# mpieva/mapping-iterative-assembler

Measured on AMD Instinct MI355X. Metric: reads aligned/sec per iteration (16.5kb mito ref, 100bp reads), higher is better.
Workload: dtype int32; 1 GPU; configs[1]: 1000000 synthetic 100 bp reads per GPU vs mt311 (16619 bp, circular), matrix flat; step = reiterate_assembly + pop_smp + cull + consensus; pass-1 coordinates = true positions; reads_per_gpu=1000000, total_reads=1000000, consensus_len=16619, bytes_per_read=182

## Files before the change

mapping-iterative-assembler_amd/csrc/mia_hip.hip:

```cpp
#include <hip/hip_runtime.h>
#include <atomic>
#include <hip/hip_ext.h>
#include <stdio.h>
#include <stdlib.h>
#include <string.h>

#include <algorithm>
#include <cmath>
#include <chrono>
#include <string>
#include <thread>
#include <vector>

#include "../../include/mia_hip.h"
#include "mia_comm.h"
#include "mia_consensus_kernels.h"
#include "mia_kernels.h"
#include "bandx_kernels.h"
#include "mia_pass1_kernels.h"
#include "mia_myers_kernels.h"
#include "mia_trim_kernels.h"
#include "mia_peak_kernels.h"
#include "mia_iter_kernels.h"

using namespace mia;

enum Stage { STG_TRACE = 0, STG_PLAIN, STG_FILTER, STG_BAND, STG_BX_PLAN, STG_BX_VALUES, STG_BX_TRACE, STG_TALLY, STG_PASS1, STG_COUNT };
static const char* const STAGE_NAMES[STG_COUNT] = {"k_align_quad", "k_align_quad_plain", "k_diag_filter", "k_band_align", "k_bx_plan",
                                                   "k_bx_values", "k_bx_trace", "k_tally_binned", "k_pass1"};

constexpr int OPEN_WGS = 1024;
constexpr int64_t OPEN_SLAB_BYTES = (int64_t)MAX_READ * 64 * 12;
constexpr int CTRL_BINS = 0;
constexpr int CTRL_HDR = (3 * N_BINS + 2 + 1) & ~1;
constexpr int CTRL_FILTER = CTRL_HDR + PH_WORDS;
constexpr int CTRL_LKN = CTRL_FILTER + 4, CTRL_CULLF = CTRL_LKN + 1, CTRL_NEV = CTRL_CULLF + 1, CTRL_TFLAGS = CTRL_NEV + 1, CTRL_FIXN = CTRL_TFLAGS + 1;
constexpr int CTRL_GENN = CTRL_FIXN + 1;
constexpr int CTRL_BXC = (CTRL_GENN + 1 + 63) & ~63;
constexpr int CTRL_WORDS = CTRL_BXC + BXC_WORDS;
constexpr int CTRL_C0 = CTRL_BINS + 3 * N_BINS, CTRL_CN = CTRL_WORDS - CTRL_C0;

#ifdef MIA_HIP_ALT_PATHS
static inline const char* alt_env(const char* name) { return getenv(name); }
#define ALT_KERNEL(k) ((const void*)(k))
#else
static inline const char* alt_env(const char*) { return nullptr; }
#define ALT_KERNEL(k) ((const void*)nullptr)
#endif

struct mia_hip_ctx {
  int device = 0;
  int32_t* d_ctrl = nullptr;
  uint32_t stage_mask = ~0u;
  hipStream_t stream = nullptr;
  hipStream_t stream2 = nullptr; hipEvent_t ev_fork = nullptr, ev_join = nullptr;
  hipStream_t stream3 = nullptr; hipEvent_t ev_join3 = nullptr;
  int32_t* d_retry2 = nullptr; int64_t retry2_cap = 0;
  uint32_t* d_bx_slabs_late = nullptr; int64_t bx_slab_late_cap = 0; int bx_late_wgs = 0;
  uint32_t* d_bx_slabs_late2 = nullptr; bool dp_aside = false;
  const int32_t* abort_if = nullptr;
  bool spec_ok = false, spec_pending = false, spec_filtered = false, spec_bx = false, spec_plain = false;
  int64_t spec_redone = 0;
  bool pend_encode = false; int32_t pend_L = 0, pend_wl = 0, pend_total = 0;
  uint32_t* d_prep_bar = nullptr; uint32_t prep_bar_count = 0; bool no_prep_fuse = false;
  KbPair* d_kbits = nullptr;
  int use_quick = 1; int64_t quick_steps = 0;
  bool direct_open_now = false;
  int32_t* d_open_list = nullptr; int64_t open_cap = 0; unsigned char* d_slabs_open = nullptr; bool use_direct_open = true; int64_t direct_open_steps = 0;
  bool spec_force = false; int32_t* d_one = nullptr;
  bool zero_copy = true;
  bool cull_scan = false, tail_scans = false, stage_markers = false;
  bool spin_wait = true;
  uint32_t ext_events = 31u; bool planner_end_signalled = false, align_end_signalled = false;
  BxCandRec* d_bx_cand2 = nullptr; int use_fine = 1;
  BxCandRec* d_bx_cand = nullptr; int64_t cand_cap = 0, cand2_cap = 0; bool plan_split = true;
  bool no_spec = false;
  bool no_side_buckets = false;
  int buckets_queued = 0;
  hipStream_t stream4 = nullptr; hipEvent_t ev_early = nullptr;
  hipEvent_t ev_snap = nullptr, ev_v1 = nullptr; uint32_t* d_bx_snap = nullptr; int split_dp_mode = 0;
  bool cull_with_records = true;
  int64_t split_dp_steps = 0;
  bool use_early = false, early_queued = false;
  int early_wgs_per_cu = 2;
  uint8_t* d_early = nullptr; int32_t* d_trec_early = nullptr; int32_t* d_order_e = nullptr; int32_t* d_fix_list = nullptr; int64_t early_cap = 0;
  int32_t* d_bucket_e = nullptr; int bucket_e_cap = 0, bucket_e_clean_nb = -1;
  int32_t* d_tally_slabs_e = nullptr; int64_t tally_slab_e_cap = 0;
  unsigned char* d_slabs_retry[3] = {nullptr, nullptr, nullptr};
  bool bx_planner_aside = false;
  bool bx_pending_join = false;
  std::string err;
// ... 227 lines not shown
    const char* npl = alt_env("MIA_HIP_NO_PLAIN");
    if (npl && atoi(npl)) ctx->use_plain = 0;
    const char* pbb = alt_env("MIA_HIP_PLAIN_BEHIND_BAND");
    if (pbb && atoi(pbb)) ctx->plain_behind_band = 1;
    const char* nf = alt_env("MIA_HIP_NO_DIAG_FILTER");
    if (nf && atoi(nf)) { ctx->use_filter = 0; ctx->use_bx = 0; }
    const char* nbd = alt_env("MIA_HIP_NO_BAND_DP");
    if (nbd && atoi(nbd)) { ctx->use_banddp = 0; ctx->use_bx = 0; }
    const char* nbx = alt_env("MIA_HIP_NO_BANDX");
    if (nbx && atoi(nbx)) ctx->use_bx = 0;
    if (const char* nl2 = alt_env("MIA_HIP_NO_LANES")) if (atoi(nl2)) ctx->use_lanes = 0;
    if (const char* bd2 = alt_env("MIA_HIP_BX_DEBUG")) ctx->bx_dbg = (uint32_t)atoi(bd2);
    if (const char* bs2 = alt_env("MIA_HIP_BX_SERIAL")) ctx->bx_serial = atoi(bs2) != 0;
    if (const char* sb2 = alt_env("MIA_HIP_NO_SIDE_BUCKETS")) ctx->no_side_buckets = atoi(sb2) != 0;
    if (const char* ns2 = alt_env("MIA_HIP_NO_SPEC")) ctx->no_spec = atoi(ns2) != 0;
    if (const char* pf2 = alt_env("MIA_HIP_NO_PREP_FUSE")) ctx->no_prep_fuse = atoi(pf2) != 0;
    if (const char* ps2 = alt_env("MIA_HIP_NO_PLAN_SPLIT")) ctx->plan_split = atoi(ps2) == 0;
    if (const char* zc = alt_env("MIA_HIP_NO_ZERO_COPY")) ctx->zero_copy = atoi(zc) == 0;
    if (const char* ef = alt_env("MIA_HIP_NO_EXT_EVENTS")) ctx->ext_events = atoi(ef) ? 0u : 31u;
    if (const char* cs = alt_env("MIA_HIP_CULL_SCAN")) ctx->cull_scan = atoi(cs) != 0;
    if (const char* sm = alt_env("MIA_HIP_STAGE_MARKERS")) ctx->stage_markers = atoi(sm) != 0;
    if (const char* ts = alt_env("MIA_HIP_TAIL_SCANS")) ctx->tail_scans = atoi(ts) != 0;
    if (const char* dop = alt_env("MIA_HIP_NO_DIRECT_OPEN")) ctx->use_direct_open = atoi(dop) == 0;
    if (const char* qp = alt_env("MIA_HIP_NO_QUICK_PLAN")) ctx->use_quick = atoi(qp) == 0 ? 1 : 0;
    if (const char* qp = alt_env("MIA_HIP_QUICK_PLAN")) ctx->use_quick = atoi(qp);
    if (const char* sw = getenv("MIA_HIP_SPIN_WAIT")) ctx->spin_wait = atoi(sw) != 0;
    if (const char* em = alt_env("MIA_HIP_EXT_EVENTS_MASK")) ctx->ext_events = (uint32_t)atoi(em);
    if (const char* st2 = alt_env("MIA_HIP_SPEC_TEST")) ctx->spec_force = atoi(st2) != 0;
    if (const char* ml = alt_env("MIA_HIP_MYERS_NO_LANES")) ctx->myers_no_lanes = atoi(ml) != 0;
    if (const char* mo = alt_env("MIA_HIP_MYERS_NO_OND")) ctx->myers_no_ond = atoi(mo) != 0;
    if (const char* fo = alt_env("MIA_HIP_FAKE_EVENT_OVERFLOW")) ctx->fake_event_overflow = atoi(fo) != 0;
    if (const char* na = alt_env("MIA_HIP_NO_AUTO_PLAIN")) ctx->no_auto_plain = atoi(na) != 0;
    const char* egs = alt_env("MIA_HIP_EAGER_SCRIPTS");
    if (egs && atoi(egs)) ctx->lazy_scripts = 0;
    const char* nwl = alt_env("MIA_HIP_NO_WILD");
    if (nwl && atoi(nwl)) ctx->use_wild = 0;
    if (const char* ne = alt_env("MIA_HIP_EARLY_TALLY")) ctx->use_early = atoi(ne) != 0;
    if (const char* ti = alt_env("MIA_HIP_TALLY_INLINE")) ctx->tally_defer = atoi(ti) == 0;
    if (const char* ss = alt_env("MIA_HIP_STRAND_SPLIT")) ctx->tally_strand_split = atoi(ss) != 0;
    if (const char* nr = alt_env("MIA_HIP_NO_TALLY_RUNS")) ctx->tally_runs = atoi(nr) == 0;
    if (const char* sd = alt_env("MIA_HIP_SPLIT_DP")) ctx->split_dp_mode = atoi(sd) != 0 ? 1 : -1;
    if (const char* ra = alt_env("MIA_HIP_NO_TALLY_RALL")) ctx->tally_rall = atoi(ra) == 0;
    if (const char* cr = alt_env("MIA_HIP_NO_CULL_RECORDS")) ctx->cull_with_records = atoi(cr) == 0;
    if (const char* tc = alt_env("MIA_HIP_TALLY_CHUNK")) { const int c = atoi(tc); if (c == 256 || c == 512 || c == 768) ctx->tally_chunk_linear = c; }
    if (const char* ew = alt_env("MIA_HIP_EARLY_WGS")) ctx->early_wgs_per_cu = atoi(ew);
    if (const char* nf = alt_env("MIA_HIP_NO_FINE")) ctx->use_fine = atoi(nf) == 0 ? 1 : 0;
// ... 398 lines not shown
  return MIA_HIP_OK;
}

#ifdef MIA_HIP_ALT_PATHS
extern "C" int mia_hip_debug_tally_kinds(mia_hip_ctx* ctx, uint64_t* out8) {
  if (!ctx || !out8) return MIA_HIP_ERR_ARG;
  HIPCHK(hipStreamSynchronize(ctx->stream));
  HIPCHK(hipMemcpyFromSymbol(out8, HIP_SYMBOL(g_tally_kinds), 8 * sizeof(uint64_t)));
  uint64_t z[8] = {0, 0, 0, 0, 0, 0, 0, 0};
  HIPCHK(hipMemcpyToSymbol(HIP_SYMBOL(g_tally_kinds), z, sizeof z));
  HIPCHK(hipMemcpyFromSymbol(out8 + 8, HIP_SYMBOL(g_tally_clk), 8 * sizeof(uint64_t)));
  HIPCHK(hipMemcpyToSymbol(HIP_SYMBOL(g_tally_clk), z, sizeof z));
  return MIA_HIP_OK;
}
extern "C" int mia_hip_debug_plan_clk(mia_hip_ctx* ctx, uint64_t* out12) {
  if (!ctx || !out12) return MIA_HIP_ERR_ARG;
  HIPCHK(hipStreamSynchronize(ctx->stream));
  static uint64_t all[64 * 16], z[64 * 16];
  HIPCHK(hipMemcpyFromSymbol(all, HIP_SYMBOL(g_plan_clk), sizeof all));
  for (int k = 0; k < 12; k++) { out12[k] = 0; for (int st = 0; st < 64; st++) out12[k] += all[st * 16 + k]; }
  HIPCHK(hipMemcpyToSymbol(HIP_SYMBOL(g_plan_clk), z, sizeof z));
  return MIA_HIP_OK;
}
#endif
extern "C" int mia_hip_bx_counters(mia_hip_ctx* ctx, uint32_t* out32) {
  if (!ctx || !out32) return MIA_HIP_ERR_ARG;
  for (int k = 0; k < 32; k++) out32[k] = ctx->bx_last[k];
  return MIA_HIP_OK;
}

extern "C" int mia_hip_plain_stats(mia_hip_ctx* ctx, int reset, double* plain_ms, int64_t* plain_launches, int64_t* reads_in, int64_t* reads_retried) {
  if (!ctx) return MIA_HIP_ERR_ARG;
  HIPCHK(hipSetDevice(ctx->device));
  drain_events(ctx);
  if (plain_ms) *plain_ms = ctx->stg[STG_PLAIN].ms;
  if (plain_launches) *plain_launches = ctx->stg[STG_PLAIN].launches;
  if (reads_in) *reads_in = ctx->plain_total;
  if (reads_retried) *reads_retried = ctx->plain_retried;
  if (reset) { ctx->stg[STG_PLAIN].ms = 0; ctx->stg[STG_PLAIN].launches = 0; ctx->plain_total = 0; ctx->plain_retried = 0; }
  return MIA_HIP_OK;
}

template <int CPL>
static hipError_t launch_window(mia_hip_ctx* ctx, int ci, const int32_t* list, int count, const int32_t* dev_range = nullptr, hipStream_t on = nullptr,
                                bool own_slabs = false, hipEvent_t stop = nullptr) {
  const int64_t slab = (int64_t)MAX_READ * 64 * CPL;
// ... 2 lines not shown
    const int cus = ctx->cus;
    if (hipOccupancyMaxActiveBlocksPerMultiprocessor(&occ, (const void*)k_align_window<CPL>, 64, 0) != hipSuccess || occ < 1) occ = 1;
    const int per_cu = ctx->grid_wgs / cus;
    ctx->window_wgs[ci] = cus * (occ < per_cu ? occ : per_cu);
  }
  int grid = (dev_range || count >= ctx->window_wgs[ci]) ? ctx->window_wgs[ci] : count;
  unsigned char* slabs = nullptr;
  if (own_slabs) {
    grid = std::min(grid, 1024);
    if (!ctx->d_slabs_retry[ci] && hipMalloc((void**)&ctx->d_slabs_retry[ci], (size_t)slab * 1024) != hipSuccess) return hipErrorOutOfMemory;
    slabs = ctx->d_slabs_retry[ci];
  } else {
    if (!ctx->d_slabs[ci]) {
      if (hipMalloc((void**)&ctx->d_slabs[ci], (size_t)slab * ctx->grid_wgs) != hipSuccess) return hipErrorOutOfMemory;
    }
    slabs = ctx->d_slabs[ci];
  }
  RefInfo ref{ctx->d_ref, ctx->L, ctx->wrap, ctx->explicit_win};
  if (stage_begin(ctx, STG_TRACE, on)) return hipErrorOutOfMemory;
  launch_k(k_align_window<CPL>, dim3(grid), dim3(64), 0, on ? on : ctx->stream, stop, ctx->rs, ref, ctx->d_pssm, ctx->packs.p[ci], list,
           count, slabs, slab, ctx->d_wide_list, ctx->d_bins + 3 * N_BINS, ctx->dbg, dev_range);
  stage_end(ctx, STG_TRACE, on);
  return hipGetLastError();
}

static int bx_join_and_retry(mia_hip_ctx* ctx) {
  if (!ctx->bx_pending_join) return MIA_HIP_OK;
  ctx->bx_pending_join = false;
  const int32_t* range = ctx->d_plan_hdr + PH_RETRY2;
  const int cols = ctx->max_len + 2 * REALIGN_BUFFER + 2;
  const bool aside = ctx->bx_planner_aside;
  if (!aside || ctx->dp_aside) HIPCHK(hipStreamWaitEvent(ctx->stream, ctx->ev_join, 0));
  HIPCHK(hipStreamWaitEvent(ctx->stream, ctx->ev_join3, 0));
  hipEvent_t stop = (aside && (ctx->ext_events & 8u)) ? ctx->ev_fork : nullptr;
  ctx->align_end_signalled = stop != nullptr;
  hipError_t e;
  if (ctx->direct_open_now) {
    RefInfo ref{ctx->d_ref, ctx->L, ctx->wrap, ctx->explicit_win};
    if (stage_begin(ctx, STG_TRACE)) return MIA_HIP_ERR_NOMEM;
    launch_k(k_align_open, dim3(OPEN_WGS), dim3(64), 0, ctx->stream, stop, ctx->rs, ref, (const int32_t*)ctx->d_pssm, ctx->packs, (const int32_t*)ctx->d_open_list,
             (const uint32_t*)(ctx->d_bx_ctr + (size_t)BXC_OPEN * BXC_STRIDE), ctx->d_slabs_open, (int64_t)OPEN_SLAB_BYTES, ctx->d_wide_list, ctx->d_bins + 3 * N_BINS, ctx->dbg,
             (const int32_t*)ctx->d_retry2, (const uint32_t*)(range + 1));
    stage_end(ctx, STG_TRACE);
    e = hipGetLastError();
    if (e != hipSuccess) { ctx->err = std::string("k_align_open launch: ") + hipGetErrorString(e); return MIA_HIP_ERR_DEVICE; }
    return MIA_HIP_OK;
  }
  e = cols <= 64 * 4 ? launch_window<4>(ctx, 0, ctx->d_retry2, 0, range, nullptr, aside, stop)
    : cols <= 64 * 8 ? launch_window<8>(ctx, 1, ctx->d_retry2, 0, range, nullptr, aside, stop)
                     : launch_window<12>(ctx, 2, ctx->d_retry2, 0, range, nullptr, aside, stop);
  if (e != hipSuccess) { ctx->err = std::string("k_align_window (band retry list) launch: ") + hipGetErrorString(e); return MIA_HIP_ERR_DEVICE; }
  if (aside) {
    if (!ctx->planner_end_signalled) HIPCHK(hipEventRecord(ctx->ev_join, ctx->stream2));
    ctx->planner_end_signalled = false;
    HIPCHK(hipStreamWaitEvent(ctx->stream, ctx->ev_join, 0));
  }
  return MIA_HIP_OK;
}

static int align_all(mia_hip_ctx* ctx);
static int early_tally_launch(mia_hip_ctx* ctx);
static bool tally_is_binned(const mia_hip_ctx* ctx);
static int comm_pre_cull_enqueue(mia_hip_ctx* ctx, const int32_t* d_wide_count);
static bool comm_pre_cull_collect(mia_hip_ctx* ctx);
// ... 245 lines not shown
      bd.cand2 = nullptr; bd.cand2_n = ctx->d_bx_ctr + (size_t)BXC_CAND2 * BXC_STRIDE;
      int64_t rejects_before = 0;
      for (int k = 1; k < BXF_KINDS; k++) rejects_before += ctx->bx_last[BXC_FAIL0 + k];
      const bool fine = split && ctx->use_fine && (ctx->use_fine > 1 || !ctx->flat || n >= 4000000 || !ctx->ref_mostly_bases || rejects_before * 20 > n);
      if (split) {
        if (n > ctx->cand_cap) {
          if (dev_alloc(ctx, &ctx->d_bx_cand, (size_t)n)) return MIA_HIP_ERR_NOMEM;
          ctx->cand_cap = n;
        }
        if (fine && n > ctx->cand2_cap) {
          if (dev_alloc(ctx, &ctx->d_bx_cand2, (size_t)n)) return MIA_HIP_ERR_NOMEM;
          ctx->cand2_cap = n;
        }
        bd.cand = ctx->d_bx_cand;
        if (fine) bd.cand2 = ctx->d_bx_cand2;
      }
      const int last_phase = split ? (fine ? 3 : 2) : 0;
      {
        int64_t lr = 0;
        for (int k = 1; k < BXF_KINDS; k++) lr += ctx->bx_last[BXC_FAIL0 + k];
        const bool many_early = !ctx->no_auto_plain && (!ctx->ref_mostly_bases || lr * 20 > n);
        planner_head_first = new_flow && ctx->deferred && many_early && !ctx->planner_beside && !(ctx->dbg & 256u);
        const bool plain_wanted = ctx->use_plain && (ctx->plain_behind_band || many_early);
        direct_open = new_flow && ctx->deferred && ctx->use_direct_open && !plain_wanted && !planner_head_first && !run_filter && !(ctx->dbg & 256u) &&
                      !(ctx->bx_dbg & (4u | 8u));
      }
      bd.open = nullptr; bd.open_n = ctx->d_bx_ctr + (size_t)BXC_OPEN * BXC_STRIDE;
      ctx->direct_open_now = direct_open;
      if (direct_open) {
        if (n > ctx->open_cap) { if (dev_alloc(ctx, &ctx->d_open_list, (size_t)n)) return MIA_HIP_ERR_NOMEM; ctx->open_cap = n; }
        if (!ctx->d_slabs_open && hipMalloc((void**)&ctx->d_slabs_open, (size_t)OPEN_SLAB_BYTES * OPEN_WGS) != hipSuccess) return MIA_HIP_ERR_NOMEM;
        bd.open = ctx->d_open_list;
        ctx->direct_open_steps++;
      }
      const bool early = ctx->deferred && new_flow && ctx->use_early && !run_filter && tally_is_binned(ctx) && n <= 4000000;
      bd.early = nullptr;
      if (early) {
        if (n > ctx->early_cap) {
          if (dev_alloc(ctx, &ctx->d_early, (size_t)n) || dev_alloc(ctx, &ctx->d_trec_early, (size_t)n * 16) || dev_alloc(ctx, &ctx->d_order_e, (size_t)n) ||
              dev_alloc(ctx, &ctx->d_fix_list, (size_t)n)) return MIA_HIP_ERR_NOMEM;
          ctx->early_cap = n;
        }
        bd.early = ctx->d_early;
      }
      if (!fine && ctx->use_fine < 2) bd.tab.maxw = 32;
      const bool split_dp = new_flow && ctx->deferred && split && last_phase >= 2 && !early && !(ctx->bx_dbg & (4u | 8u)) && ctx->split_dp_mode > 0;
      bd.snap = nullptr;
      if (split_dp) {
        if (!ctx->d_bx_snap && dev_alloc(ctx, &ctx->d_bx_snap, (size_t)(2 * BX_NCLS))) return MIA_HIP_ERR_NOMEM;
        bd.snap = ctx->d_bx_snap;
        ctx->split_dp_steps++;
      }
      const bool quick = split && new_flow && !run_filter && !early && !split_dp && want_bits && !(ctx->bx_dbg & 32u) && bd.umax != nullptr &&
                         (!fine || n >= 2000000 || ctx->use_quick > 1);
// ... 1094 lines not shown
```

mapping-iterative-assembler_amd/csrc/mia_hip_iterate.inc:

```

constexpr int PRE_WORDS = 8;
#define COLLCHK(call)                                                                                  \
  do {                                                                                                 \
    const int r_ = (call);                                                                             \
    if (r_ != MIA_HIP_OK) {                                                                            \
      const char* t_ = ctx->coll.error ? ctx->coll.error(ctx->coll.user) : nullptr;                    \
      ctx->err = std::string(#call) + ": " + (t_ && *t_ ? t_ : "collective failed");                   \
      return r_;                                                                                       \
    }                                                                                                  \
  } while (0)

static int comm_attach_table(mia_hip_ctx* ctx, const mia_hip_collectives& t) {
  if (dev_alloc(ctx, &ctx->d_gather, (size_t)PRE_WORDS * t.n_ranks)) return MIA_HIP_ERR_NOMEM;
  ctx->coll = t;
  ctx->coll_name = t.name ? t.name : "";
  ctx->coll.name = t.name ? ctx->coll_name.c_str() : nullptr;
  ctx->comm = true; ctx->comm_ranks = t.n_ranks; ctx->comm_rank = t.rank;
  ctx->h_gather.assign((size_t)PRE_WORDS * t.n_ranks, 0);
  ctx->ev_pad = 0;
  return MIA_HIP_OK;
}

extern "C" int mia_hip_comm_init(mia_hip_ctx* ctx, const void* id128, int32_t n_ranks, int32_t rank) {
  if (!ctx || !id128 || n_ranks < 1 || n_ranks > 256 || rank < 0 || rank >= n_ranks) return MIA_HIP_ERR_ARG;
// ... 137 lines not shown
  }
  ctx->ref_mostly_bases = n_other * 50 <= L;
  ctx->ref_few_n = n_other * 500 <= L;
  ctx->kh_entries = 0;
  if (n_other && ctx->use_wild) {
    int64_t e = 0;
    int k = 0;
    auto other = [&](int j) { return base_code(new_ref[j < L ? j : j - L]) > 3 ? 1 : 0; };
    for (int pq = 0; pq < wrap; pq++) {
      k += other(pq);
      if (pq >= DF_K) k -= other(pq - DF_K);
      if (pq >= DF_K - 1 && k <= BX_WILD) e += (int64_t)1 << (2 * k);
    }
    ctx->kh_entries = e > ((int64_t)1 << 24) ? 0 : e;
  }
  if (total > ctx->ref_cap) {
    if (dev_alloc(ctx, &ctx->d_ref, (size_t)total * 2)) return MIA_HIP_ERR_NOMEM;
    ctx->ref_cap = total * 2;
  }
  if (L > ctx->ascii_cap) {
    if (dev_alloc(ctx, &ctx->d_ascii, (size_t)L * 2)) return MIA_HIP_ERR_NOMEM;
    ctx->ascii_cap = (int64_t)L * 2;
  }
  if (ctx->h_pin && (size_t)L <= mia_hip_ctx::PIN_BYTES - mia_hip_ctx::PIN_MISC) {
    HIPCHK(hipStreamSynchronize(ctx->stream));
    memcpy(ctx->h_pin + mia_hip_ctx::PIN_MISC, new_ref, (size_t)L);
    if (ctx->zero_copy) ctx->ascii_src = reinterpret_cast<const char*>(ctx->h_pin + mia_hip_ctx::PIN_MISC);
    else { HIPCHK(hipMemcpyAsync(ctx->d_ascii, ctx->h_pin + mia_hip_ctx::PIN_MISC, (size_t)L, hipMemcpyHostToDevice, ctx->stream)); ctx->ascii_src = ctx->d_ascii; }
  } else {
    HIPCHK(hipMemcpyAsync(ctx->d_ascii, new_ref, (size_t)L, hipMemcpyHostToDevice, ctx->stream));
    ctx->ascii_src = ctx->d_ascii;
  }
  ctx->pend_encode = true; ctx->pend_L = L; ctx->pend_wl = wl; ctx->pend_total = total;
  if (ctx->rs.n == 0) { encode_now(ctx); HIPCHK(hipGetLastError()); }
  const bool dbg_steps = alt_env("MIA_HIP_ITER_DEBUG") != nullptr;
  static const bool host_laps = getenv("MIA_HIP_TIMING") != nullptr;
  const auto lap_t0 = std::chrono::steady_clock::now();
  auto checkpoint = [&](const char* what) {
    if (dbg_steps) { hipError_t e = hipStreamSynchronize(ctx->stream); fprintf(stderr, "[mia_hip_iterate] %s: %s\n", what, hipGetErrorString(e)); fflush(stderr); }
    if (host_laps) fprintf(stderr, "[mia_hip_iterate host] %-20s %8.2f ms\n", what, std::chrono::duration<double, std::milli>(std::chrono::steady_clock::now() - lap_t0).count());
  };
  checkpoint("reference");
  ctx->L = L; ctx->wrap = wrap; ctx->have_ref = true; ctx->explicit_win = 0;
  const int64_t n = ctx->rs.n;
  const int W = ctx->comm_ranks;
  if (ctx->comm && n == 0) { ctx->err = "iterate: every rank of a sharded run needs reads"; return MIA_HIP_ERR_ARG; }
// ... 269 lines not shown
```

mapping-iterative-assembler_amd/csrc/mia_kernels.h:

```cpp
#pragma once
#include <hip/hip_runtime.h>
#include <stdint.h>

#include "align_body.h"
#include "align_body_quad.h"
#include "align_body_quad_plain.h"
#include "diag_filter.h"
#include "band_body.h"
#include "mia_layout.h"
#include "wave_dev.h"

namespace mia {

constexpr int N_CPL = 3;
constexpr int BIN_WIDE = N_CPL;
constexpr int BIN_QUAD0 = BIN_WIDE + 1;
constexpr int N_BINS = BIN_QUAD0 + MAX_READ + 1;
constexpr int SUB_LDS_BYTES = MAX_READ * 10;

struct ReadSet {
  int64_t n;
  const uint8_t* packed;
  const uint32_t* roff;
  const uint16_t* len;
  const uint8_t* rc;
  const uint8_t* sk;
  int32_t* as;
// ... 335 lines not shown
    a.pk = pk;
    a.lds_sub = 0;
    a.trace_stride = (uint32_t)((l1 + 3) & ~3);
    a.cols_out = rs.cols + (int64_t)i * rs.stride;
    a.dbg = dbg;
    AlignResult r = WindowAligner<DevWave, CPL>::run(wave, a);
    if (wave.lane() == 0) {
      if (r.status & ST_ESCAPE) {
        int p = atomicAdd(wide_count, 1);
        wide_list[p] = i;
      } else {
        rs.score[i] = r.score;
        rs.refstart[i] = s;
        rs.abr[i] = (int16_t)r.abr;
        rs.as[i] = r.abc + s;
        rs.ae[i] = r.aec + s;
      }
      rs.status[i] = r.status;
    }
    wave.lds_fence();
  }
}

__global__ __launch_bounds__(64) void k_align_open(ReadSet rs, RefInfo ref, const int32_t* pssm2, PackSet ps, const int32_t* list, const uint32_t* count_p,
                                                    unsigned char* trace_slabs, int64_t slab_bytes, int32_t* wide_list, int32_t* wide_count, uint32_t dbg,
                                                    const int32_t* list_b, const uint32_t* count_b_p) {
  __shared__ __attribute__((aligned(16))) unsigned char lds_raw[SUB_LDS_BYTES];
  const int count_a = (int)*count_p, count = count_a + (list_b ? (int)*count_b_p : 0);
  __builtin_amdgcn_s_setprio(3);
  DevWave wave(lds_raw, trace_slabs + (int64_t)blockIdx.x * slab_bytes);
  for (int w = blockIdx.x; w < count; w += gridDim.x) {
    const int i = w < count_a ? list[w] : list_b[w - count_a];
    if (!rs.sk[i]) { if (wave.lane() == 0) rs.status[i] = ST_SKIPPED; continue; }
    AlignArgs a;
    int s, l1;
    const int len2 = rs.len[i];
    read_window(ref, rs.as[i], rs.ae[i], len2, &s, &l1);
    const int ci = classify(len2, l1, ps, 0);
    if (ci == BIN_WIDE) {
      if (wave.lane() == 0) { const int q = atomicAdd(wide_count, 1); wide_list[q] = i; }
      continue;
    }
    a.ref_codes = ref.codes;
    a.ref_start = s;
    a.len1 = l1;
    a.read_packed = rs.packed + rs.roff[i];
    a.len2 = len2;
    a.pssm = pssm2 + (rs.rc[i] ? PSSM_WORDS : 0);
    a.sg5 = 1;
    a.pk = ps.p[ci];
    a.lds_sub = 0;
    a.trace_stride = (uint32_t)((l1 + 3) & ~3);
    a.cols_out = rs.cols + (int64_t)i * rs.stride;
    a.dbg = dbg;
    AlignResult r;
    if (ci == 0) r = WindowAligner<DevWave, 4>::run(wave, a);
    else if (ci == 1) r = WindowAligner<DevWave, 8>::run(wave, a);
    else r = WindowAligner<DevWave, 12>::run(wave, a);
    if (wave.lane() == 0) {
      if (r.status & ST_ESCAPE) {
        const int q = atomicAdd(wide_count, 1);
        wide_list[q] = i;
      } else {
        rs.score[i] = r.score;
        rs.refstart[i] = s;
        rs.abr[i] = (int16_t)r.abr;
        rs.as[i] = r.abc + s;
        rs.ae[i] = r.aec + s;
      }
      rs.status[i] = r.status;
    }
    wave.lds_fence();
  }
}

__global__ __launch_bounds__(64, 4) void k_align_quad(ReadSet rs, RefInfo ref, const int32_t* pssm2, PackParams pk, const int32_t* list,
                                                    int32_t n_quads, unsigned char* trace_slabs, int64_t slab_bytes,
                                                    int32_t* wide_list, int32_t* wide_count, int32_t* retry_list, int32_t* retry_count,
                                                    int32_t band, uint32_t dbg, const int32_t* dev_range) {
  extern __shared__ __attribute__((aligned(16))) unsigned char lds_raw[];
  if (dev_range) { list += dev_range[0]; n_quads = dev_range[1]; }
  __builtin_amdgcn_s_setprio(1);
  DevWave wave(lds_raw, trace_slabs + (int64_t)blockIdx.x * slab_bytes);
  for (int qd = blockIdx.x; qd < n_quads; qd += gridDim.x) {
    QuadArgs a;
    int idx[Q_G];
    a.ref_codes = ref.codes;
    a.packed = rs.packed;
    a.pssm2 = pssm2;
    a.pk = pk;
    a.lds_sub = 0;
    a.slab_group = (uint32_t)(slab_bytes / Q_G);
    a.dbg = dbg;
    a.band = band;
    a.len2 = 1;
// ... 197 lines not shown
```

mapping-iterative-assembler_amd/csrc/wave_dev.h:

```cpp
#pragma once
#include <hip/hip_runtime.h>
#include <stdint.h>

#include "mia_layout.h"

namespace mia {

constexpr int DPP_ROW_SHR = 0x110;
constexpr int DPP_WAVE_SHR1 = 0x138;
constexpr int DPP_ROW_BCAST15 = 0x142;
constexpr int DPP_ROW_BCAST31 = 0x143;

struct DevWave {
  typedef uint32_t U;
  typedef bool M;
  unsigned char* lds;
  unsigned char* trace;

  __device__ __forceinline__ DevWave(unsigned char* l, unsigned char* t) : lds(l), trace(t) {}

  __device__ __forceinline__ U lane() const { return __builtin_amdgcn_mbcnt_hi(~0u, __builtin_amdgcn_mbcnt_lo(~0u, 0u)); }

  __device__ __forceinline__ U shr1(U x, U fill) const {
    return (U)__builtin_amdgcn_update_dpp((int)fill, (int)x, DPP_WAVE_SHR1, 0xF, 0xF, false);
// ... 122 lines not shown
  __device__ __forceinline__ U lds_r32m(U off, M ok) const { return ok ? *reinterpret_cast<const uint32_t*>(lds + off) : 0u; }
  __device__ __forceinline__ static U gload_u32(const uint32_t* p, U i, M ok) { return ok ? p[i] : 0u; }
  __device__ __forceinline__ static void gstore_u32(uint32_t* p, U i, U v, M ok) { if (ok) p[i] = v; }
  __device__ __forceinline__ U tr_r16(U off, M ok) const {
    return ok ? (U)__hip_atomic_load(reinterpret_cast<const uint16_t*>(trace + off), __ATOMIC_RELAXED, __HIP_MEMORY_SCOPE_AGENT) : 0u;
  }
  __device__ __forceinline__ void tr_w32(U off, U v, M ok) const { if (ok) *reinterpret_cast<uint32_t*>(trace + off) = v; }
  __device__ __forceinline__ U tr_r8(U off, M ok) const {
    return ok ? (U)__hip_atomic_load(trace + off, __ATOMIC_RELAXED, __HIP_MEMORY_SCOPE_AGENT) : 0u;
  }
  __device__ __forceinline__ void tr_fence() const {
    __builtin_amdgcn_fence(__ATOMIC_RELEASE, "workgroup");
    __builtin_amdgcn_wave_barrier();
    __builtin_amdgcn_fence(__ATOMIC_ACQUIRE, "workgroup");
  }
  __device__ __forceinline__ void sched_fence() const { __builtin_amdgcn_sched_barrier(0); }
  __device__ __forceinline__ void lds_fence() const {
    __builtin_amdgcn_fence(__ATOMIC_RELEASE, "workgroup");
    __builtin_amdgcn_wave_barrier();
    __builtin_amdgcn_fence(__ATOMIC_ACQUIRE, "workgroup");
  }
};

}
```

Baseline: 1.388 billion reads/s.

## Align open reads with a 256-thread workgroup and LDS trace matrix

k_align_open now runs as a 256-thread workgroup. Short reads in the narrowest bin (up to 154 rows) are aligned by a new GroupAligner, which spreads reference columns across four waves, passes row carries between waves through a small LDS exchange buffer, and keeps the traceback matrix in LDS instead of global slabs. Other reads fall back to the single-wave aligner on wave 0. The grid is sized from occupancy, and slabs are allocated according to the maximum read length. In return, every row adds a workgroup barrier, LDS use per block grows, and three waves sit idle on the fallback path.

```diff
diff --git a/mapping-iterative-assembler_amd/csrc/align_body_wg.h b/mapping-iterative-assembler_amd/csrc/align_body_wg.h
--- /dev/null
+++ b/mapping-iterative-assembler_amd/csrc/align_body_wg.h
@@ -0,0 +1,180 @@
+#pragma once
+#include "align_body.h"
+
+namespace mia {
+
+constexpr int WG_COLS = 256;
+constexpr int WG_MAX_ROWS = 154;
+
+template <class W>
+MIA_HD static inline __attribute__((always_inline)) void wg_traceback(W& w, const AlignArgs& a, uint32_t stride, AlignResult& res) {
+  typedef typename W::U U;
+  typedef typename W::M M;
+  const U lane = w.lane();
+  int r = res.aer, c = res.aec;
+  uint32_t status = ST_OK;
+  int aln_cols = 0;
+  for (int guard = 0; guard < 4 * MAX_READ + 8; guard++) {
+    U ri = U((uint32_t)r) - lane, ci = U((uint32_t)c) - lane;
+    M inside = (lane <= (uint32_t)r) & (lane <= (uint32_t)c);
+    U tb = w.tr_r8(ri * stride + ci, inside);
+    U ty = tb >> 6, ln = tb & 63u;
+    M colgap0 = (ty == U(TR_COLGAP)) & (ln + 1u == ci) & (ln < U(TR_LEN_SAT));
+    M rowgap0 = (ty == U(TR_ROWGAP)) & (ln + 1u == ri) & (ln < U(TR_LEN_SAT));
+    M plain_diag = (ty == U(TR_DIAG)) | colgap0 | rowgap0;
+    M terminal = (ri == U(0u)) | (ci == U(0u)) | (ty == U(TR_START));
+    M stop_here = (!inside) | terminal | (!plain_diag);
+    uint64_t bal = w.ballot(stop_here);
+    int f = bal ? __builtin_ctzll(bal) : WAVE;
+    int npairs = f < WAVE ? f + 1 : WAVE;
+    if (f < WAVE && !w.lane_bit(inside, f)) npairs = f;
+    w.gstore_i16(a.cols_out, ri, ci, lane < (uint32_t)npairs);
+    aln_cols += npairs;
+    if (f == WAVE) { r -= WAVE; c -= WAVE; continue; }
+    const uint32_t fty = w.lane_val(ty, f), fln = w.lane_val(ln, f);
+    const bool fterm = w.lane_bit(terminal, f);
+    const int fr = r - f, fc = c - f;
+    if (fterm) { res.abr = fr; res.abc = fc; break; }
+    if (fln >= TR_LEN_SAT) { status |= ST_ESCAPE; res.abr = fr; res.abc = fc; break; }
+    if (fty == TR_COLGAP) {
+      r = fr - 1; c = fc - 1 - (int)fln;
+      aln_cols += (int)fln;
+    } else {
+      U rr = U((uint32_t)(fr - 1)) - lane;
+      w.gstore_i16(a.cols_out, rr, U((uint32_t)(uint16_t)COL_INSERT), lane < fln);
+      r = fr - 1 - (int)fln; c = fc - 1;
+      aln_cols += (int)fln;
+    }
+  }
+  for (int r0 = 0; r0 < res.abr; r0 += WAVE) {
+    U rr = lane + (uint32_t)r0;
+    w.gstore_i16(a.cols_out, rr, U((uint32_t)(uint16_t)COL_CLIP), rr < (uint32_t)res.abr);
+  }
+  if (aln_cols > 2 * MAX_READ) status |= ST_TOO_LONG;
+  res.status = status;
+}
+
+template <class G>
+struct GroupAligner {
+  typedef typename G::U U;
+  typedef typename G::M M;
+  static constexpr int IB = PackBits<4>::IB, SH = PackBits<4>::SH;
+  static constexpr uint32_t IDXM = PackBits<4>::IDXM;
+
+  struct Prev { U s, rr, p63, p62; };
+  MIA_HD static inline __attribute__((always_inline)) Prev gather(G& w, int buf, const U& wid, uint32_t freshb, const U& unav) {
+    U x0[4], x1[4], x2[4];
+    w.xw_get4(buf, 0, x0);
+    w.xw_get4(buf, 1, x1);
+    w.xw_get4(buf, 2, x2);
+    const M is0 = wid == 0u, is1 = wid == 1u, is2 = wid == 2u;
+    Prev p;
+    p.s = w.sel(is0, U(freshb), w.sel(is1, x0[0], w.sel(is2, x1[0], x2[0])));
+    p.rr = w.sel(is0, unav, w.sel(is1, x0[1], w.sel(is2, x1[1], x2[1])));
+    const U m01 = w.umax(x0[2], x1[2]), m012 = w.umax(m01, x2[2]);
+    p.p63 = w.sel(is0, unav, w.sel(is1, x0[2], w.sel(is2, m01, m012)));
+    p.p62 = w.sel(is0, unav, w.sel(is1, x0[3], w.sel(is2, w.umax(x0[2], x1[3]), w.umax(m01, x2[3]))));
+    return p;
+  }
+
+  MIA_HD static inline __attribute__((always_inline)) AlignResult run(G& w, const AlignArgs& a) {
+    const uint32_t OFF = (uint32_t)a.pk.off;
+    const uint32_t UNAV = ((uint32_t)a.pk.unavail << SH) | IDXM;
+    const U col = w.tid(), lane = w.lane(), wid = w.wave_id();
+    const M lane0 = lane == 0u;
+    const int len1 = a.len1, len2 = a.len2;
+    const uint32_t RS2 = (uint32_t)((len2 + 1) & ~1) * 2u;
+
+    for (int e0 = 0; e0 < len2 * 5; e0 += WG_COLS) {
+      U e = col + (uint32_t)e0;
+      M ok = e < (uint32_t)(len2 * 5);
+      U r = w.udiv5(e);
+      U c1 = e - r * 5u;
+      U byte = w.gload_u8(a.read_packed, r >> 1, ok);
+      U c2 = (byte >> ((r & 1u) << 2)) & 15u;
+      U d = w.depth(r, (uint32_t)len2);
+      U v = w.gload_i32(a.pssm, (d * 5u + c1) * 5u + c2, ok);
+      w.lds_w16(U(a.lds_sub) + c1 * RS2 + r * 2u, v, ok);
+    }
+    const M in = col < (uint32_t)len1;
+    const U code = w.sel(in, w.gload_u8(a.ref_codes, U((uint32_t)a.ref_start) + col, in), U(4u));
+    const U sub_addr = U(a.lds_sub) + code * RS2;
+    const U KC = (U(0u) - ((U((uint32_t)GOP) + (col - 1u) * (uint32_t)GEP) << SH)) + (TR_COLGAP << IB) + (col - 1u - IDXM);
+    const U QC = ((col * (uint32_t)GEP) << SH) + (U(IDXM) - col);
+    const uint32_t WDC = TR_DIAG << IB;
+    const U unav = U(UNAV);
+    w.stamp(2);
+    w.barrier();
+    w.stamp(3);
+
+    U pw = w.lds_r32(sub_addr);
+    U Sb = w.sext_lo(pw) + OFF;
+    U q = (Sb << SH) + QC;
+    U pend = (Sb << SH) + IDXM;
+    U rrun = unav;
+    w.tr_w8(col, U(TR_DIAG << 6));
+    U s = w.scan_max(q);
+    U e1raw = w.shr1(s, unav);
+    w.xw_put4(0, Sb, rrun, s, e1raw);
+    w.barrier();
+    w.stamp(4);
+
+    for (int r = 1; r < len2; r++) {
+      const int32_t fresh = a.sg5 ? -(GOP + GEP * (r + 1)) : 0;
+      const uint32_t freshb = (uint32_t)(fresh + (int32_t)OFF);
+      const uint32_t WS = freshb << SH;
+      const uint32_t KR = (0u - ((uint32_t)(GOP + GEP * (r - 1)) << SH)) + (TR_ROWGAP << IB) + ((uint32_t)(r - 1) - IDXM);
+      const uint32_t RK = ((uint32_t)(GEP * r) << SH) + (IDXM - (uint32_t)r);
+      const bool hi = (r & 1) != 0;
+      if (!hi) pw = w.lds_r32(sub_addr + (uint32_t)r * 2u);
+      const Prev p = gather(w, (r - 1) & 1, wid, freshb, unav);
+      const U dleft = w.shr1(Sb, p.s);
+      const U rleft = w.shr1(rrun, p.rr);
+      const U e1 = w.sel(lane0, p.p63, e1raw);
+      const U e2 = w.shr1(e1, p.p62);
+      const U excl = w.umax(e2, w.sel(lane0, unav, p.p63));
+      const U Wd = (dleft << SH) + WDC;
+      const U Wc = excl + KC;
+      const U Wr = rleft + KR;
+      const U m3 = w.umax3(Wd, Wc, Wr);
+      const U best = w.umax(m3, U(WS));
+      const U sub = hi ? w.sext_hi(pw) : w.sext_lo(pw);
+      const U Snew = (best >> SH) + w.sel(m3 < WS, U(0u), sub);
+      w.tr_w8(U((uint32_t)r * (uint32_t)WG_COLS) + col, (((best >> IB) & 3u) << 6) | w.umin(best & IDXM, U(TR_LEN_SAT)));
+      rrun = w.umax(rrun, pend);
+      pend = (Snew << SH) + RK;
+      q = (Snew << SH) + QC;
+      Sb = Snew;
+      s = w.scan_max(q);
+      e1raw = w.shr1(s, unav);
+      w.xw_put4(r & 1, Sb, rrun, s, e1raw);
+      w.barrier();
+    }
+    w.stamp(5);
+
+    AlignResult res;
+    res.abr = 0;
+    res.abc = 0;
+    res.aer = len2 - 1;
+    {
+      const U key = w.sel(in, (Sb << 8) + (U(255u) - col), U(0u));
+      const U km = w.scan_max(key);
+      const int buf = len2 & 1;
+      w.xw_put4(buf, km, km, km, km);
+      w.barrier();
+      U x0[4], x1[4], x2[4], x3[4];
+      w.xw_get4(buf, 0, x0); w.xw_get4(buf, 1, x1); w.xw_get4(buf, 2, x2); w.xw_get4(buf, 3, x3);
+      const uint32_t k = w.uniform(w.umax(w.umax(x0[0], x1[0]), w.umax(x2[0], x3[0])));
+      res.score = (int32_t)((k >> 8) - OFF);
+      res.aec = (int32_t)(255u - (k & 255u));
+    }
+    w.stamp(6);
+
+    res.status = ST_OK;
+    if (w.first_wave()) wg_traceback(w.wave0(), a, (uint32_t)WG_COLS, res);
+    w.stamp(7);
+    return res;
+  }
+};
+
+}
diff --git a/mapping-iterative-assembler_amd/csrc/mia_hip.hip b/mapping-iterative-assembler_amd/csrc/mia_hip.hip
--- a/mapping-iterative-assembler_amd/csrc/mia_hip.hip
+++ b/mapping-iterative-assembler_amd/csrc/mia_hip.hip
@@ -29,8 +29,6 @@
 static const char* const STAGE_NAMES[STG_COUNT] = {"k_align_quad", "k_align_quad_plain", "k_diag_filter", "k_band_align", "k_bx_plan",
                                                    "k_bx_values", "k_bx_trace", "k_tally_binned", "k_pass1"};
 
-constexpr int OPEN_WGS = 1024;
-constexpr int64_t OPEN_SLAB_BYTES = (int64_t)MAX_READ * 64 * 12;
 constexpr int CTRL_BINS = 0;
 constexpr int CTRL_HDR = (3 * N_BINS + 2 + 1) & ~1;
 constexpr int CTRL_FILTER = CTRL_HDR + PH_WORDS;
@@ -67,6 +65,7 @@
   int use_quick = 1; int64_t quick_steps = 0;
   bool direct_open_now = false;
   int32_t* d_open_list = nullptr; int64_t open_cap = 0; unsigned char* d_slabs_open = nullptr; bool use_direct_open = true; int64_t direct_open_steps = 0;
+  int open_wgs = 0; int64_t open_slab_bytes = 0, open_slab_cap = 0; uint32_t open_dbg = 0; bool open_overflow = false;
   bool spec_force = false; int32_t* d_one = nullptr;
   bool zero_copy = true;
   bool cull_scan = false, tail_scans = false, stage_markers = false;
@@ -340,6 +339,8 @@
     if (const char* sm = alt_env("MIA_HIP_STAGE_MARKERS")) ctx->stage_markers = atoi(sm) != 0;
     if (const char* ts = alt_env("MIA_HIP_TAIL_SCANS")) ctx->tail_scans = atoi(ts) != 0;
     if (const char* dop = alt_env("MIA_HIP_NO_DIRECT_OPEN")) ctx->use_direct_open = atoi(dop) == 0;
+    if (const char* ow = alt_env("MIA_HIP_OPEN_WG")) if (atoi(ow) == 0) ctx->open_dbg |= OPEN_DBG_ONE_WAVE;
+    if (const char* oc = alt_env("MIA_HIP_OPEN_CLK")) if (atoi(oc)) ctx->open_dbg |= OPEN_DBG_CLK;
     if (const char* qp = alt_env("MIA_HIP_NO_QUICK_PLAN")) ctx->use_quick = atoi(qp) == 0 ? 1 : 0;
     if (const char* qp = alt_env("MIA_HIP_QUICK_PLAN")) ctx->use_quick = atoi(qp);
     if (const char* sw = getenv("MIA_HIP_SPIN_WAIT")) ctx->spin_wait = atoi(sw) != 0;
@@ -784,6 +785,14 @@
   HIPCHK(hipMemcpyToSymbol(HIP_SYMBOL(g_plan_clk), z, sizeof z));
   return MIA_HIP_OK;
 }
+extern "C" int mia_hip_debug_open_clk(mia_hip_ctx* ctx, uint64_t* out64) {
+  if (!ctx || !out64) return MIA_HIP_ERR_ARG;
+  HIPCHK(hipStreamSynchronize(ctx->stream));
+  static uint64_t z[4 * 16];
+  HIPCHK(hipMemcpyFromSymbol(out64, HIP_SYMBOL(g_open_clk), sizeof z));
+  HIPCHK(hipMemcpyToSymbol(HIP_SYMBOL(g_open_clk), z, sizeof z));
+  return MIA_HIP_OK;
+}
 #endif
 extern "C" int mia_hip_bx_counters(mia_hip_ctx* ctx, uint32_t* out32) {
   if (!ctx || !out32) return MIA_HIP_ERR_ARG;
@@ -832,6 +841,26 @@
            count, slabs, slab, ctx->d_wide_list, ctx->d_bins + 3 * N_BINS, ctx->dbg, dev_range);
   stage_end(ctx, STG_TRACE, on);
   return hipGetLastError();
+}
+
+static int open_setup(mia_hip_ctx* ctx) {
+  if (!ctx->use_direct_open) return MIA_HIP_OK;
+  if (!ctx->open_wgs) {
+    int occ = 0;
+    if (hipOccupancyMaxActiveBlocksPerMultiprocessor(&occ, (const void*)k_align_open, 256, 0) != hipSuccess || occ < 1) occ = 1;
+    ctx->open_wgs = ctx->cus * std::min(occ, 3);
+  }
+  const int64_t slab = (int64_t)std::max(ctx->max_len, 1) * 64 * 12;
+  if (slab * ctx->open_wgs > ctx->open_slab_cap) {
+    size_t free0 = 0, free1 = 0, total = 0;
+    const bool log = alt_env("MIA_HIP_OPEN_CLK") != nullptr;
+    if (log) (void)hipMemGetInfo(&free0, &total);
+    if (dev_alloc(ctx, &ctx->d_slabs_open, (size_t)(slab * ctx->open_wgs))) return MIA_HIP_ERR_NOMEM;
+    ctx->open_slab_cap = slab * ctx->open_wgs;
+    if (log) { (void)hipMemGetInfo(&free1, &total); fprintf(stderr, "[open_setup] grid %d x 256, slab %lld bytes: device memory in use +%.1f MB\n", ctx->open_wgs, (long long)slab, ((double)free0 - (double)free1) / 1e6); }
+  }
+  ctx->open_slab_bytes = slab;
+  return MIA_HIP_OK;
 }
 
 static int bx_join_and_retry(mia_hip_ctx* ctx) {
@@ -848,8 +877,8 @@
   if (ctx->direct_open_now) {
     RefInfo ref{ctx->d_ref, ctx->L, ctx->wrap, ctx->explicit_win};
     if (stage_begin(ctx, STG_TRACE)) return MIA_HIP_ERR_NOMEM;
-    launch_k(k_align_open, dim3(OPEN_WGS), dim3(64), 0, ctx->stream, stop, ctx->rs, ref, (const int32_t*)ctx->d_pssm, ctx->packs, (const int32_t*)ctx->d_open_list,
-             (const uint32_t*)(ctx->d_bx_ctr + (size_t)BXC_OPEN * BXC_STRIDE), ctx->d_slabs_open, (int64_t)OPEN_SLAB_BYTES, ctx->d_wide_list, ctx->d_bins + 3 * N_BINS, ctx->dbg,
+    launch_k(k_align_open, dim3(ctx->open_wgs), dim3(256), 0, ctx->stream, stop, ctx->rs, ref, (const int32_t*)ctx->d_pssm, ctx->packs, (const int32_t*)ctx->d_open_list,
+             (const uint32_t*)(ctx->d_bx_ctr + (size_t)BXC_OPEN * BXC_STRIDE), ctx->d_slabs_open, ctx->open_slab_bytes, ctx->d_wide_list, ctx->d_bins + 3 * N_BINS, (ctx->dbg & 7u) | ctx->open_dbg,
              (const int32_t*)ctx->d_retry2, (const uint32_t*)(range + 1));
     stage_end(ctx, STG_TRACE);
     e = hipGetLastError();
@@ -1141,14 +1170,15 @@
         const bool many_early = !ctx->no_auto_plain && (!ctx->ref_mostly_bases || lr * 20 > n);
         planner_head_first = new_flow && ctx->deferred && many_early && !ctx->planner_beside && !(ctx->dbg & 256u);
         const bool plain_wanted = ctx->use_plain && (ctx->plain_behind_band || many_early);
+        if ((int64_t)ctx->bx_last[BXC_OPEN] > ctx->open_wgs) ctx->open_overflow = true;
+        else if (lr <= ctx->open_wgs) ctx->open_overflow = false;
         direct_open = new_flow && ctx->deferred && ctx->use_direct_open && !plain_wanted && !planner_head_first && !run_filter && !(ctx->dbg & 256u) &&
-                      !(ctx->bx_dbg & (4u | 8u));
+                      !(ctx->bx_dbg & (4u | 8u)) && ctx->d_slabs_open && !ctx->open_overflow;
       }
       bd.open = nullptr; bd.open_n = ctx->d_bx_ctr + (size_t)BXC_OPEN * BXC_STRIDE;
       ctx->direct_open_now = direct_open;
       if (direct_open) {
         if (n > ctx->open_cap) { if (dev_alloc(ctx, &ctx->d_open_list, (size_t)n)) return MIA_HIP_ERR_NOMEM; ctx->open_cap = n; }
-        if (!ctx->d_slabs_open && hipMalloc((void**)&ctx->d_slabs_open, (size_t)OPEN_SLAB_BYTES * OPEN_WGS) != hipSuccess) return MIA_HIP_ERR_NOMEM;
         bd.open = ctx->d_open_list;
         ctx->direct_open_steps++;
       }
diff --git a/mapping-iterative-assembler_amd/csrc/mia_hip_iterate.inc b/mapping-iterative-assembler_amd/csrc/mia_hip_iterate.inc
--- a/mapping-iterative-assembler_amd/csrc/mia_hip_iterate.inc
+++ b/mapping-iterative-assembler_amd/csrc/mia_hip_iterate.inc
@@ -183,6 +183,7 @@
     if (dev_alloc(ctx, &ctx->d_ascii, (size_t)L * 2)) return MIA_HIP_ERR_NOMEM;
     ctx->ascii_cap = (int64_t)L * 2;
   }
+  if (open_setup(ctx)) return MIA_HIP_ERR_NOMEM;
   if (ctx->h_pin && (size_t)L <= mia_hip_ctx::PIN_BYTES - mia_hip_ctx::PIN_MISC) {
     HIPCHK(hipStreamSynchronize(ctx->stream));
     memcpy(ctx->h_pin + mia_hip_ctx::PIN_MISC, new_ref, (size_t)L);
diff --git a/mapping-iterative-assembler_amd/csrc/mia_kernels.h b/mapping-iterative-assembler_amd/csrc/mia_kernels.h
--- a/mapping-iterative-assembler_amd/csrc/mia_kernels.h
+++ b/mapping-iterative-assembler_amd/csrc/mia_kernels.h
@@ -3,6 +3,7 @@
 #include <stdint.h>
 
 #include "align_body.h"
+#include "align_body_wg.h"
 #include "align_body_quad.h"
 #include "align_body_quad_plain.h"
 #include "diag_filter.h"
@@ -384,23 +385,42 @@
   }
 }
 
-__global__ __launch_bounds__(64) void k_align_open(ReadSet rs, RefInfo ref, const int32_t* pssm2, PackSet ps, const int32_t* list, const uint32_t* count_p,
-                                                    unsigned char* trace_slabs, int64_t slab_bytes, int32_t* wide_list, int32_t* wide_count, uint32_t dbg,
-                                                    const int32_t* list_b, const uint32_t* count_b_p) {
-  __shared__ __attribute__((aligned(16))) unsigned char lds_raw[SUB_LDS_BYTES];
+constexpr uint32_t OPEN_DBG_ONE_WAVE = 1u << 29, OPEN_DBG_CLK = 1u << 28;
+constexpr int OPEN_XW_BYTES = 2 * 4 * 16;
+constexpr int OPEN_LDS_BYTES = SUB_LDS_BYTES + OPEN_XW_BYTES + WG_MAX_ROWS * WG_COLS;
+#ifdef MIA_HIP_ALT_PATHS
+__device__ unsigned long long g_open_clk[4 * 16];
+#endif
+__global__ __launch_bounds__(256) void k_align_open(ReadSet rs, RefInfo ref, const int32_t* pssm2, PackSet ps, const int32_t* list, const uint32_t* count_p,
+                                                     unsigned char* trace_slabs, int64_t slab_bytes, int32_t* wide_list, int32_t* wide_count, uint32_t dbg,
+                                                     const int32_t* list_b, const uint32_t* count_b_p) {
+  __shared__ __attribute__((aligned(16))) unsigned char lds_raw[OPEN_LDS_BYTES];
   const int count_a = (int)*count_p, count = count_a + (list_b ? (int)*count_b_p : 0);
   __builtin_amdgcn_s_setprio(3);
+  const bool wave0 = threadIdx.x < 64u;
+  unsigned long long* clk = nullptr;
+#ifdef MIA_HIP_ALT_PATHS
+  __shared__ unsigned long long clk_s[9];
+  if (dbg & OPEN_DBG_CLK) clk = clk_s;
+#endif
   DevWave wave(lds_raw, trace_slabs + (int64_t)blockIdx.x * slab_bytes);
+  DevGroup group(lds_raw, reinterpret_cast<uint4*>(lds_raw + SUB_LDS_BYTES), lds_raw + SUB_LDS_BYTES + OPEN_XW_BYTES, clk);
   for (int w = blockIdx.x; w < count; w += gridDim.x) {
+#ifdef MIA_HIP_ALT_PATHS
+    if (clk && threadIdx.x == 0) { for (int k = 1; k < 9; k++) clk[k] = 0; clk[0] = __builtin_amdgcn_s_memtime(); }
+#endif
     const int i = w < count_a ? list[w] : list_b[w - count_a];
-    if (!rs.sk[i]) { if (wave.lane() == 0) rs.status[i] = ST_SKIPPED; continue; }
+    if (!rs.sk[i]) { if (threadIdx.x == 0) rs.status[i] = ST_SKIPPED; continue; }
     AlignArgs a;
     int s, l1;
     const int len2 = rs.len[i];
     read_window(ref, rs.as[i], rs.ae[i], len2, &s, &l1);
-    const int ci = classify(len2, l1, ps, 0);
+    int ci = classify(len2, l1, ps, 0);
+    a.trace_stride = (uint32_t)((l1 + 3) & ~3);
+    const bool as_group = ci == 0 && len2 <= WG_MAX_ROWS && !(dbg & OPEN_DBG_ONE_WAVE);
+    if (ci != BIN_WIDE && !as_group && (int64_t)len2 * a.trace_stride > slab_bytes) ci = BIN_WIDE;
     if (ci == BIN_WIDE) {
-      if (wave.lane() == 0) { const int q = atomicAdd(wide_count, 1); wide_list[q] = i; }
+      if (threadIdx.x == 0) { const int q = atomicAdd(wide_count, 1); wide_list[q] = i; }
       continue;
     }
     a.ref_codes = ref.codes;
@@ -412,14 +432,18 @@
     a.sg5 = 1;
     a.pk = ps.p[ci];
     a.lds_sub = 0;
-    a.trace_stride = (uint32_t)((l1 + 3) & ~3);
     a.cols_out = rs.cols + (int64_t)i * rs.stride;
-    a.dbg = dbg;
-    AlignResult r;
-    if (ci == 0) r = WindowAligner<DevWave, 4>::run(wave, a);
-    else if (ci == 1) r = WindowAligner<DevWave, 8>::run(wave, a);
-    else r = WindowAligner<DevWave, 12>::run(wave, a);
-    if (wave.lane() == 0) {
+    a.dbg = dbg & 7u;
+    group.stamp(1);
+    AlignResult r{};
+    if (as_group) r = GroupAligner<DevGroup>::run(group, a);
+    else if (wave0) {
+      if (ci == 0) r = WindowAligner<DevWave, 4>::run(wave, a);
+      else if (ci == 1) r = WindowAligner<DevWave, 8>::run(wave, a);
+      else r = WindowAligner<DevWave, 12>::run(wave, a);
+      group.stamp(7);
+    }
+    if (threadIdx.x == 0) {
       if (r.status & ST_ESCAPE) {
         const int q = atomicAdd(wide_count, 1);
         wide_list[q] = i;
@@ -431,8 +455,17 @@
         rs.ae[i] = r.aec + s;
       }
       rs.status[i] = r.status;
-    }
-    wave.lds_fence();
+#ifdef MIA_HIP_ALT_PATHS
+      if (clk) {
+        clk[8] = __builtin_amdgcn_s_memtime();
+        const int row = (as_group ? 0 : 2) + ((r.aec - r.abc) != (len2 - 1 - r.abr) ? 1 : 0);
+        for (int k = 1; k < 9; k++) if (!clk[k]) clk[k] = clk[k - 1];
+        for (int k = 0; k < 8; k++) atomicAdd(&g_open_clk[row * 16 + k], clk[k + 1] - clk[k]);
+        atomicAdd(&g_open_clk[row * 16 + 15], 1ull);
+      }
+#endif
+    }
+    __syncthreads();
   }
 }
 
diff --git a/mapping-iterative-assembler_amd/csrc/wave_dev.h b/mapping-iterative-assembler_amd/csrc/wave_dev.h
--- a/mapping-iterative-assembler_amd/csrc/wave_dev.h
+++ b/mapping-iterative-assembler_amd/csrc/wave_dev.h
@@ -168,4 +168,57 @@
   }
 };
 
+struct DevWaveLdsTrace : DevWave {
+  const unsigned char* ltrace;
+  __device__ __forceinline__ DevWaveLdsTrace(unsigned char* l, const unsigned char* t) : DevWave(l, nullptr), ltrace(t) {}
+  __device__ __forceinline__ U tr_r8(U off, M ok) const { return ok ? (U)ltrace[off] : 0u; }
+};
+
+struct DevGroup {
+  typedef uint32_t U;
+  typedef bool M;
+  unsigned char* lds;
+  unsigned char* ltrace;
+  uint4* xw;
+  unsigned long long* clk;
+  DevWaveLdsTrace w0;
+
+  __device__ __forceinline__ DevGroup(unsigned char* sub, uint4* words, unsigned char* trace, unsigned long long* stamps)
+      : lds(sub), ltrace(trace), xw(words), clk(stamps), w0(sub, trace) {}
+
+  __device__ __forceinline__ U tid() const { return threadIdx.x; }
+  __device__ __forceinline__ U lane() const { return threadIdx.x & 63u; }
+  __device__ __forceinline__ U wave_id() const { return (U)__builtin_amdgcn_readfirstlane((int)(threadIdx.x >> 6)); }
+  __device__ __forceinline__ bool first_wave() const { return threadIdx.x < 64u; }
+  __device__ __forceinline__ DevWaveLdsTrace& wave0() { return w0; }
+  __device__ __forceinline__ void barrier() const { __syncthreads(); }
+  __device__ __forceinline__ void stamp(int k) const { if (clk && threadIdx.x == 0) clk[k] = __builtin_amdgcn_s_memtime(); }
+  __device__ __forceinline__ static uint32_t uniform(U v) { return (uint32_t)__builtin_amdgcn_readfirstlane((int)v); }
+
+  __device__ __forceinline__ U shr1(U x, U fill) const {
+    return (U)__builtin_amdgcn_update_dpp((int)fill, (int)x, DPP_WAVE_SHR1, 0xF, 0xF, false);
+  }
+  __device__ __forceinline__ U scan_max(U v) const { return w0.scan_max(v); }
+  __device__ __forceinline__ static U umax(U a, U b) { return a > b ? a : b; }
+  __device__ __forceinline__ static U umin(U a, U b) { return a < b ? a : b; }
+  __device__ __forceinline__ static U umax3(U a, U b, U c) { return umax(umax(a, b), c); }
+  __device__ __forceinline__ static U sel(M c, U a, U b) { return c ? a : b; }
+  __device__ __forceinline__ static U sext_lo(U x) { return DevWave::sext_lo(x); }
+  __device__ __forceinline__ static U sext_hi(U x) { return DevWave::sext_hi(x); }
+  __device__ __forceinline__ static U udiv5(U e) { return e / 5u; }
+  __device__ __forceinline__ static U depth(U row, uint32_t len) { return (U)sm_depth((int)row, (int)len); }
+  __device__ __forceinline__ static U gload_u8(const uint8_t* p, U i, M ok) { return ok ? (U)p[i] : 0u; }
+  __device__ __forceinline__ static U gload_i32(const int32_t* p, U i, M ok) { return ok ? (U)p[i] : 0u; }
+  __device__ __forceinline__ void lds_w16(U off, U v, M ok) const { if (ok) *reinterpret_cast<uint16_t*>(lds + off) = (uint16_t)v; }
+  __device__ __forceinline__ U lds_r32(U off) const { return *reinterpret_cast<const uint32_t*>(lds + off); }
+  __device__ __forceinline__ void tr_w8(U off, U v) const { ltrace[off] = (unsigned char)v; }
+  __device__ __forceinline__ void xw_put4(int buf, U a, U b, U c, U d) const {
+    if ((threadIdx.x & 63u) == 63u) xw[buf * 4 + (threadIdx.x >> 6)] = make_uint4(a, b, c, d);
+  }
+  __device__ __forceinline__ void xw_get4(int buf, int k, U out[4]) const {
+    const uint4 v = xw[buf * 4 + k];
+    out[0] = v.x; out[1] = v.y; out[2] = v.z; out[3] = v.w;
+  }
+};
+
 }
```

New measurement: 1.397 billion reads/s (median of 6 runs). No clear change (+0.6%).
